# gerbenvoshol/fqzcomp5

Hardware: AMD Instinct MI355X
Metric: input MB/s encode+decode, 100MB blocks, -3 and -5; bit-exact vs CPU (higher is better)
Workload: dtype u8

## Files before the change

fqzcomp5_amd/csrc/block.cpp:

```cpp
#include <atomic>
#include <cstdio>
#include <algorithm>
#include <cstdlib>
#include <cstring>
#include <exception>
#include <functional>
#include <thread>
#include <deque>
#include <memory>
#include <vector>

#include "../../include/fqz5_block.h"
#include "rans_codec.hpp"
#include "fqz_codec.hpp"
#include "seq_codec.hpp"
#include "seq_cm.h"
#include "lzp_codec.hpp"
#include "names.hpp"
#include "host_dec.hpp"
#include "rans_format.hpp"

namespace fqz5 {

GpuCtx &gpu();
// ... 1033 lines not shown
                DecompressReq r;
                r.h_in = hs;
                r.d_in = secs[i].in + 9;
                r.in_size = clen;
                r.out_cap = rsz;
                r.d_out = g.arena.alloc_n<uint8_t>(size_t(rsz) + 1);
                LzpDecReq z;
                z.d_in = r.d_out;
                z.d_out = secs[i].out;
                z.cap = ulen;
                lzp_rans.push_back(reqs.size());
                reqs.push_back(r);
                who.push_back(-1);
                lzd.push_back(z);
                who_lzp.push_back(i);
                continue;
            }
            if (h[0] != 0) continue;
            DecompressReq r;
            r.h_in = h + 9;
            r.d_in = secs[i].in + 9;
            r.in_size = clen;
            r.out_cap = ulen;
            r.d_out = secs[i].out;
            reqs.push_back(r);
            who.push_back(i);
        }
        const double t1 = now_ms();
        const int hmode = host_decode_mode();
        std::vector<int> fqz_kind(fqz.size(), host::CK_FQZ), fqz_src(fqz.size(), -1);
        for (size_t k = 0; k < fqz.size(); k++) {
            const FqzDecReq &f = fqz[k];
            uint32_t tl = 0;
            const int vk = varint_get(f.h_in, f.h_in + f.in_size, &tl);
            if (vk > 0 && size_t(vk) + 1 < f.in_size && (f.h_in[vk + 1] & 8u) && f.d_seq) {
                fqz_kind[k] = host::CK_FQZ_SEQ;
                for (size_t m = 0; m < seqd.size(); m++)
                    if (seqd[m].d_out == f.d_seq) fqz_src[k] = int(m);
            }
        }
        std::vector<uint64_t> chain_n;
        std::vector<int> chain_kind;
        for (const SeqDecReq &q : seqd) { chain_n.push_back(q.n); chain_kind.push_back(host::CK_SEQ); }
        for (size_t k = 0; k < fqz.size(); k++) { chain_n.push_back(fqz[k].out_cap); chain_kind.push_back(fqz_kind[k]); }
        const std::vector<char> on = host::place(hmode, chain_n, chain_kind, 0);
        std::vector<char> seq_on_host(on.begin(), on.begin() + seqd.size()),
                          fqz_on_host(on.begin() + seqd.size(), on.end());
        for (size_t k = 0; k < fqz.size(); k++)
            if (fqz_src[k] >= 0 && seq_on_host[size_t(fqz_src[k])]) fqz_on_host[k] = 1;
        g_chains_host += uint64_t(std::count(seq_on_host.begin(), seq_on_host.end(), 1) +
                                  std::count(fqz_on_host.begin(), fqz_on_host.end(), 1));
        g_chains_gpu += uint64_t(std::count(seq_on_host.begin(), seq_on_host.end(), 0) +
                                 std::count(fqz_on_host.begin(), fqz_on_host.end(), 0));
        struct HostChain { uint8_t *buf = nullptr; size_t cap = 0, n = 0; int sec = -1; bool ok = false; };
        std::vector<HostChain> hc;
        std::vector<size_t> hc_idx;
        std::vector<int> hc_kind;
        for (size_t k = 0; k < seqd.size(); k++) {
            if (!seq_on_host[k]) continue;
            HostChain c;
            c.cap = c.n = seqd[k].n;
            c.buf = g.staging.alloc(c.cap + 1);
            c.sec = who_seq[k];
            hc.push_back(c);
            hc_idx.push_back(k);
            hc_kind.push_back(host::CK_SEQ);
        }
        for (size_t k = 0; k < fqz.size(); k++) {
            if (!fqz_on_host[k]) continue;
            HostChain c;
            c.cap = fqz[k].out_cap;
            c.buf = g.staging.alloc(c.cap + 1);
            c.sec = who_fqz[k];
            hc.push_back(c);
            hc_idx.push_back(k);
            hc_kind.push_back(fqz_kind[k]);
        }
        auto timed = [](int kind, bool gpu, uint64_t n, const std::function<bool()> &fn) {
            const double a = now_ns();
            const bool ok = fn();
            if (ok) host::measured(kind, gpu, n, now_ns() - a);
            return ok;
        };
        host::Jobs hjobs;
        std::vector<size_t> early_h;
        for (size_t j = 0; j < hc.size(); j++)
            if (hc_kind[j] != host::CK_FQZ_SEQ) early_h.push_back(j);
        hjobs.start(early_h.size(), [&](size_t t) {
            const size_t j = early_h[t];
            HostChain &c = hc[j];
            if (hc_kind[j] == host::CK_SEQ) {
                const SeqDecReq &q = seqd[hc_idx[j]];
                c.ok = timed(host::CK_SEQ, false, q.n, [&] {
                    return host::seq_decode(seq_h[hc_idx[j]], q.in_size, q.lens, q.nrec, q.both, q.k,
                                            c.buf, q.n) == 0;
                });
            } else {
                const FqzDecReq &f = fqz[hc_idx[j]];
                c.ok = timed(host::CK_FQZ, false, c.cap, [&] {
                    return host::fqz_decode(f.h_in, f.in_size, c.buf, c.cap, &c.n, nullptr, 0, nullptr, 0) == 0;
                });
            }
        });
        double t_names_up = 0;
        GpuCtx *gn = nullptr;
        std::unique_ptr<HedgeShare> nshare;
        host::Task tn;
        if (!nd.empty()) {
            gn = &gpu_aux(AUX_NAMES);
            nshare = std::make_unique<HedgeShare>(size_t(g.cus));
            tn = on_ctx(*gn, "decode_sections", t0, [&] {
                names_decode_batch(*gn, nd, [&](size_t k) {
                    if (nd[k].ok && nd[k].u_len)
                        FQZ5_HIP(hipMemcpyAsync(secs[who_name[k]].out, nd[k].names,
                                                nd[k].u_len, hipMemcpyHostToDevice, gn->stream));
                });
                gn->sync();
                if (trace) t_names_up = now_ms();
            });
        }
        std::vector<FqzDecReq> fqz_early;
        std::vector<size_t> early_of;
        std::vector<char> is_early(fqz.size(), 0);
        uint64_t early_longest = 0;
        for (size_t k = 0; k < fqz.size(); k++) {
            if (fqz_on_host[k] || fqz_kind[k] == host::CK_FQZ_SEQ) continue;
            fqz_early.push_back(fqz[k]);
            early_of.push_back(k);
            is_early[k] = 1;
            early_longest = std::max<uint64_t>(early_longest, fqz[k].out_cap);
        }
        GpuCtx *gf = nullptr;
        host::Task tf;
        if (!fqz_early.empty()) {
            gf = &gpu_aux(AUX_FQZ);
            tf = on_ctx(*gf, "decode_sections", t0, [&] {
                timed(host::CK_FQZ, true, early_longest, [&] { fqz_decode_batch(*gf, fqz_early); return true; });
            });
        }
        std::vector<SeqDecReq> seq_gpu;
        std::vector<size_t> seq_gpu_of;
        uint64_t seq_longest = 0;
        for (size_t m = 0; m < seqd.size(); m++)
            if (!seq_on_host[m]) {
                seq_gpu.push_back(seqd[m]);
                seq_gpu_of.push_back(m);
                seq_longest = std::max<uint64_t>(seq_longest, seqd[m].n);
            }
        GpuCtx *gs = nullptr;
        host::Task ts;
        if (!seq_gpu.empty()) {
            gs = &gpu_aux(AUX_SEQ0);
            ts = on_ctx(*gs, "decode_sections", t0, [&] {
                timed(host::CK_SEQ, true, seq_longest, [&] { seq_decode_batch(*gs, seq_gpu); return true; });
            });
        }
        host::CoreBudget cores;
        cores.core_ns.assign(size_t(host::threads()) - std::min(size_t(host::threads()), hjobs.running()), 0.0);
        decompress_batch(g, reqs, &cores);
        const double t_rans = trace ? now_ms() : 0;
        if (trace)
            std::fprintf(stderr, "decode_sections: %zu bytes to host in %.1f ms, rANS %.1f ms\n", tot,
                         t1 - t0, now_ms() - t1);
        if (!lzd.empty()) {
            std::vector<LzpDecReq> run;
            std::vector<int> run_who;
            for (size_t k = 0; k < lzd.size(); k++) {
                const DecompressReq &r = reqs[lzp_rans[k]];
                if (!r.ok) continue;
                lzd[k].in_len = r.out_size;
                run.push_back(lzd[k]);
                run_who.push_back(who_lzp[k]);
            }
            lzp_decode_batch(g, run);
            for (size_t k = 0; k < run.size(); k++) {
                fqz5_section_result &R = res[run_who[k]];
                R.status = run[k].ok ? 0 : -1;
                R.usize = run[k].out_len;
            }
        }
        ts.join();
        for (size_t i = 0; i < seq_gpu.size(); i++) seqd[seq_gpu_of[i]] = seq_gpu[i];
        {
            std::vector<FqzDecReq> late;
            std::vector<size_t> late_of;
            uint64_t longest = 0;
            for (size_t k = 0; k < fqz.size(); k++)
                if (!is_early[k] && !fqz_on_host[k]) {
                    late.push_back(fqz[k]);
                    late_of.push_back(k);
                    longest = std::max<uint64_t>(longest, fqz[k].out_cap);
                }
            if (!late.empty()) {
                timed(host::CK_FQZ_SEQ, true, longest, [&] { fqz_decode_batch(g, late); return true; });
                for (size_t k = 0; k < late.size(); k++) fqz[late_of[k]] = late[k];
            }
        }
        tf.join();
        for (size_t k = 0; k < fqz_early.size(); k++) fqz[early_of[k]] = fqz_early[k];
        if (!hc.empty()) {
            hjobs.join();
            std::vector<std::vector<const uint8_t *>> recp(hc.size());
            for (size_t j = 0; j < hc.size(); j++) {
                if (hc_kind[j] != host::CK_FQZ_SEQ) continue;
                const FqzDecReq &f = fqz[hc_idx[j]];
                const uint8_t *bases = nullptr;
                bool host_src = false;
                for (size_t m = 0; m < hc.size(); m++)
                    if (hc_kind[m] == host::CK_SEQ && secs[hc[m].sec].out == f.d_seq) {
                        bases = hc[m].ok ? hc[m].buf : nullptr;
                        host_src = true;
                    }
                uint64_t nb = 0;
                for (int r = 0; r < f.nrec; r++) nb += f.lens[r];
                if (!bases) {
                    uint8_t *b = g.staging.alloc(nb + 1);
                    if (!host_src) g.download(b, f.d_seq, nb);
                    else std::memset(b, 0, nb + 1);
                    bases = b;
                }
                recp[j].resize(size_t(std::max(f.nrec, 1)));
                uint64_t o = 0;
                for (int r = 0; r < f.nrec; r++) {
                    recp[j][size_t(r)] = bases + o;
                    o += f.lens[r];
                }
            }
            g.sync();
            host::Jobs hb;
            std::vector<size_t> late;
            for (size_t j = 0; j < hc.size(); j++)
                if (hc_kind[j] == host::CK_FQZ_SEQ) late.push_back(j);
            hb.start(late.size(), [&](size_t t) {
                HostChain &c = hc[late[t]];
                const FqzDecReq &f = fqz[hc_idx[late[t]]];
                c.ok = timed(host::CK_FQZ_SEQ, false, c.cap, [&] {
                    return host::fqz_decode(f.h_in, f.in_size, c.buf, c.cap, &c.n, nullptr, 0,
                                            recp[late[t]].data(), f.nrec) == 0;
                });
            });
            hb.join();
            for (HostChain &c : hc) {
                fqz5_section_result &R = res[c.sec];
                R.status = c.ok ? 0 : -1;
                R.usize = uint32_t(c.n);
                if (c.ok && c.n)
                    FQZ5_HIP(hipMemcpyAsync(secs[c.sec].out, c.buf, c.n, hipMemcpyHostToDevice, g.stream));
            }
        }
        const double t_hc = trace ? now_ms() : 0;
        tn.join();
        nshare.reset();
        const double t_nj = trace ? now_ms() : 0;
        for (size_t k = 0; k < nd.size(); k++) {
            fqz5_section_result &R = res[who_name[k]];
            if (!nd[k].ok) continue;
            R.status = 0;
            R.usize = nd[k].u_len;
        }
        for (size_t k = 0; k < reqs.size(); k++) {
            if (who[k] < 0) continue;
            fqz5_section_result &R = res[who[k]];
            R.status = reqs[k].ok ? 0 : -1;
            R.usize = reqs[k].out_size;
        }
        for (size_t k = 0; k < seqd.size(); k++) {
            if (seq_on_host[k]) continue;
            fqz5_section_result &R = res[who_seq[k]];
            R.status = seqd[k].ok ? 0 : -1;
            R.usize = seqd[k].n;
        }
        for (size_t k = 0; k < fqz.size(); k++) {
            if (fqz_on_host[k]) continue;
            fqz5_section_result &R = res[who_fqz[k]];
            R.status = fqz[k].ok ? 0 : -1;
            R.usize = uint32_t(fqz[k].out_size);
        }
        g.reset();
        if (gn) gn->reset();
        if (gf) gf->reset();
        if (gs) gs->reset();
        if (trace) {
            std::fprintf(stderr, "decode_sections: from its start: rANS done %.1f, host chains joined "
                         "%.1f, names uploaded %.1f, names joined %.1f, reset %.1f ms\n", t_rans - t0,
                         t_hc - t0, t_names_up ? t_names_up - t0 : -1.0, t_nj - t0, now_ms() - t0);
        }
        return 0;
    } catch (const std::exception &e) {
        fqz5_set_error(e.what());
        try { gpu().reset(); } catch (...) {}
        try { gpu_aux_reset_all(); } catch (...) {}
        return -1;
    }
}

}
```

fqzcomp5_amd/csrc/host_sched.cpp:

```cpp
#include <sched.h>
#include <algorithm>
#include <cstdlib>

#include "../../include/fqz5_mi355x.h"
#include "host_sched.hpp"

namespace fqz5 {
namespace host {

namespace {
constexpr double HOST_RANS_O0_NS = 1.0, HOST_RANS_O1_NS = 1.4;
constexpr double HOST_RANS_ENC_O0_NS = 0.65, HOST_RANS_ENC_O1_NS = 0.85;
std::atomic<double> g_ns[CK_N][2] = {{{30.0}, {330.0}}, {{16.0}, {180.0}}, {{24.0}, {400.0}},
                                     {{HOST_RANS_O0_NS}, {13.6}}, {{HOST_RANS_O1_NS}, {18.4}},
                                     {{HOST_RANS_ENC_O0_NS}, {4.6}}, {{HOST_RANS_ENC_O1_NS}, {4.6}}};
}

double chain_ns(int kind, bool gpu) { return g_ns[kind][gpu ? 1 : 0].load(std::memory_order_relaxed); }

void chain_measured(int kind, bool gpu, double ns) {
    if (!(ns > 0.0) || kind < 0 || kind >= CK_N) return;
    std::atomic<double> &a = g_ns[kind][gpu ? 1 : 0];
    double cur = a.load(std::memory_order_relaxed);
    while (!a.compare_exchange_weak(cur, 0.5 * cur + 0.5 * ns, std::memory_order_relaxed)) {}
// ... 38 lines not shown
}

std::vector<char> place(int mode, const std::vector<uint64_t> &n, const std::vector<int> &kind,
                        uint64_t min_n, const std::vector<double> *core_ns, std::vector<double> *committed) {
    std::vector<char> on(n.size(), 0);
    if (mode == 0 || (core_ns && core_ns->empty())) return on;
    if (mode != 2) {
        for (size_t i = 0; i < on.size(); i++) on[i] = mode == 1 || i % 2 == 0;
        return on;
    }
    std::vector<size_t> at;
    std::vector<uint64_t> ln;
    std::vector<int> lk;
    for (size_t i = 0; i < n.size(); i++)
        if (n[i] >= min_n) { at.push_back(i); ln.push_back(n[i]); lk.push_back(kind[i]); }
    const std::vector<char> p = plan(ln, lk, core_ns ? int(core_ns->size()) : threads(), core_ns, committed);
    for (size_t k = 0; k < at.size(); k++) on[at[k]] = p[k];
    return on;
}

int cores_of_rank() {
    int n = 0;
    cpu_set_t set;
    CPU_ZERO(&set);
    if (sched_getaffinity(0, sizeof set, &set) == 0) n = CPU_COUNT(&set);
    if (n <= 0) n = int(std::max(1u, std::thread::hardware_concurrency()));
    if (const char *e = std::getenv("LOCAL_WORLD_SIZE")) {
        const int w = std::atoi(e);
        if (w > 1) n /= w;
    }
    if (const char *e = std::getenv("OMP_NUM_THREADS")) {
        const int o = std::atoi(e);
        if (o > 0) n = std::min(n, o);
    }
    return std::max(1, n);
}

int threads() {
    static const int n = [] {
        if (const char *e = std::getenv("FQZ5_HOST_THREADS")) return std::max(1, std::atoi(e));
        return std::min(16, cores_of_rank());
    }();
    return n;
}

bool step_trace() {
    static const bool on = std::getenv("FQZ5_STEP_TRACE") != nullptr;
    return on;
}

void Jobs::start(size_t n, std::function<void(size_t)> fn, size_t max_threads, size_t grain, size_t callers) {
    fn_ = std::move(fn);
    n_ = n;
    grain_ = std::max<size_t>(grain, 1);
    next_ = 0;
    size_t t = std::min((n + grain_ - 1) / grain_, size_t(threads()));
    if (max_threads) t = std::min(t, max_threads);
    for (size_t k = callers; k < t; k++) th_.emplace_back([this] { work(); });
}

void Jobs::work() noexcept {
    for (size_t i; (i = next_.fetch_add(grain_)) < n_;) {
        try {
            for (size_t k = i; k < std::min(n_, i + grain_); k++) fn_(k);
        } catch (...) {
            std::lock_guard<std::mutex> lk(mu_);
            if (!err_) err_ = std::current_exception();
        }
    }
}

void Jobs::join() {
    for (auto &t : th_) t.join();
    th_.clear();
    std::exception_ptr e;
    std::swap(e, err_);
    if (e) std::rethrow_exception(e);
}

Jobs::~Jobs() {
    for (auto &t : th_) t.join();
}

void parallel_for(size_t n, const std::function<void(size_t)> &fn, size_t grain, size_t serial_below) {
    if (n < serial_below || threads() == 1) {
        for (size_t i = 0; i < n; i++) fn(i);
        return;
    }
    Jobs j;
    j.start(n, fn, 0, grain, 1);
    j.work();
    j.join();
}

}
}

extern "C" void fqz5_host_plan(const uint64_t *n, const int *kind, int count, int threads,
                               const double *core_ns, char *on_host) {
    using namespace fqz5;
    const std::vector<uint64_t> nv(n, n + count);
    const std::vector<int> kv(kind, kind + count);
    std::vector<double> cores;
    if (core_ns) cores.assign(core_ns, core_ns + threads);
    const std::vector<char> on = host::plan(nv, kv, threads, core_ns ? &cores : nullptr);
    std::copy(on.begin(), on.end(), on_host);
}
```

fqzcomp5_amd/csrc/host_sched.hpp:

```cpp
#pragma once
#include <time.h>
#include <atomic>
#include <chrono>
#include <cstddef>
#include <cstdint>
#include <exception>
#include <functional>
#include <memory>
#include <mutex>
#include <thread>
#include <utility>
#include <vector>

namespace fqz5 {
namespace host {

int threads();
int cores_of_rank();

enum ChainKind { CK_SEQ = 0, CK_FQZ = 1, CK_FQZ_SEQ = 2, CK_RANS_O0 = 3, CK_RANS_O1 = 4,
                 CK_RANS_ENC_O0 = 5, CK_RANS_ENC_O1 = 6, CK_N };
double chain_ns(int kind, bool gpu);
void chain_measured(int kind, bool gpu, double ns_per_symbol);
std::vector<char> plan(const std::vector<uint64_t> &n, const std::vector<int> &kind, int threads,
                       const std::vector<double> *core_ns = nullptr,
                       std::vector<double> *committed = nullptr);

constexpr uint64_t CHAIN_MIN = 1u << 20;
void measured(int kind, bool gpu, uint64_t n, double ns);

std::vector<char> place(int mode, const std::vector<uint64_t> &n, const std::vector<int> &kind,
                        uint64_t min_n, const std::vector<double> *core_ns = nullptr,
                        std::vector<double> *committed = nullptr);

struct CoreBudget {
    std::vector<double> core_ns;
};

class Jobs {
  public:
    void start(size_t n, std::function<void(size_t)> fn, size_t max_threads = 0, size_t grain = 1,
               size_t callers = 0);
    void work() noexcept;
    void join();
    size_t running() const { return th_.size(); }
    ~Jobs();

  private:
    std::function<void(size_t)> fn_;
    size_t n_ = 0, grain_ = 1;
    std::atomic<size_t> next_{0};
    std::mutex mu_;
    std::exception_ptr err_;
    std::vector<std::thread> th_;
};

class Task {
  public:
    Task() = default;
    explicit Task(std::function<void()> fn) {
        if (!fn) return;
        err_ = std::make_unique<std::exception_ptr>();
        th_ = std::thread([fn = std::move(fn), e = err_.get()] {
            try {
                fn();
            } catch (...) {
                *e = std::current_exception();
            }
        });
    }
    Task(Task &&) = default;
    Task &operator=(Task &&o) {
        wait();
        err_ = std::move(o.err_);
        th_ = std::move(o.th_);
        return *this;
    }
    bool running() const { return th_.joinable(); }
    void join() {
        wait();
        if (err_ && *err_) std::rethrow_exception(std::exchange(*err_, nullptr));
    }
    ~Task() { wait(); }

  private:
    void wait() { if (th_.joinable()) th_.join(); }
    std::unique_ptr<std::exception_ptr> err_;
    std::thread th_;
};

void parallel_for(size_t n, const std::function<void(size_t)> &fn, size_t grain, size_t serial_below);

bool step_trace();
inline double now_ns() {
    return std::chrono::duration<double, std::nano>(
               std::chrono::steady_clock::now().time_since_epoch()).count();
}
inline double now_ms() { return now_ns() * 1e-6; }
inline double thread_cpu_ns() {
    timespec t;
    if (clock_gettime(CLOCK_THREAD_CPUTIME_ID, &t)) return 0;
    return double(t.tv_sec) * 1e9 + double(t.tv_nsec);
}

}
}
```

fqzcomp5_amd/csrc/names.cpp:

```cpp
#include <algorithm>
#include <condition_variable>
#include <cstdio>
#include <cstdlib>
#include <cstring>
#include <exception>
#include <mutex>
#include <thread>

#include "host_lzp.hpp"
#include "names.hpp"
#include "rans_format.hpp"

namespace fqz5 {

namespace {
void put32(uint8_t *p, uint32_t v) { std::memcpy(p, &v, 4); }
uint32_t get32(const uint8_t *p) { uint32_t v; std::memcpy(&v, p, 4); return v; }

void on_threads(size_t n, const std::function<void(size_t)> &fn) { host::parallel_for(n, fn, 1, 2); }
using host::now_ms;
using host::step_trace;
}

void name_prepare(const uint8_t *h, uint32_t name_len, int strat, int level, NameEnc &E,
                  bool pipelined) {
    name_split(h, name_len, strat, level, E);
    name_tokenise(E, pipelined, nullptr);
}

void name_tokenise(NameEnc &E, bool pipelined, const T3Found *found) {
    if (E.strat == 0) return;
    E.tok_ok = tok3_tokenise(E.ids.data(), int(E.ids.size()), E.level, 0, E.tok, pipelined, found);
}

void name_split(const uint8_t *h, uint32_t name_len, int strat, int level, NameEnc &E) {
    E = NameEnc();
    E.strat = strat;
    E.level = level;
    E.name_len = name_len;
    if (strat == 0) return;
    if (strat == 1) {
        E.ids.assign(h, h + name_len);
        return;
    }
    E.ids.resize(name_len + 1);
    E.comments.resize(name_len + 1);
    char *cp1 = E.ids.data(), *cp2 = E.comments.data();
    const char *nb = reinterpret_cast<const char *>(h);
    uint32_t i = 0;
    while (i < name_len) {
        uint32_t j, w1end = 0, w2start = 0, w2end = 0;
        int f = 0;
        for (j = i; j < name_len; j++) {
            if (nb[j] == '\0') {
                w2end = j;
                break;
            }
            if (!w2start && (nb[j] == ' ' || nb[j] == '\t')) {
                w1end = j;
                w2start = j + 1;
                f |= 4;
            }
        }
        if (!w1end) w1end = j;
        if (!w2end) w2end = j;
        if (w2start) f |= nb[w2start - 1] == ' ' ? 0 : 8;
        if (w1end > 1 && nb[w1end - 2] == '/') {
            if (nb[w1end - 1] == '1') f |= 1, w1end -= 2;
            else if (nb[w1end - 1] == '2') f |= 3, w1end -= 2;
        }
        E.flag.push_back(uint8_t(f));
        std::memcpy(cp1, nb + i, w1end - i);
        cp1[w1end - i] = 0;
        cp1 += w1end - i + 1;
        if (w2start) {
            std::memcpy(cp2, nb + w2start, w2end - w2start);
            cp2[w2end - w2start] = 0;
            cp2 += w2end - w2start + 1;
        }
        i = j + 1;
    }
    E.ids.resize(size_t(cp1 - E.ids.data()));
    E.comments.resize(size_t(cp2 - E.comments.data()));
}
// ... 376 lines not shown
    D.flags.assign(u_lenf, 0);
    while (cp < cp_end) {
        while (cp1 < cp1_end && cp < cp_end && *cp1) *cp++ = *cp1++;
        cp1++;
        int flag = 0;
        if (cpf < cpf_end) flag = *cpf++;
        if ((flag & 1) && cp + 1 < cp_end) {
            *cp++ = '/';
            *cp++ = (flag & 2) ? '2' : '1';
        }
        if ((flag & 4) && cp < cp_end) *cp++ = (flag & 8) ? '\t' : ' ';
        if (cp2) {
            while (cp2 < cp2_end && cp < cp_end && *cp2) *cp++ = *cp2++;
            cp2++;
        }
        if (rec < int(u_lenf)) D.flags[size_t(rec)] = (flag & 3) == 3 ? 128u : 0u;
        rec++;
        if (cp == last_cp) break;
        if (cp < cp_end) *cp++ = 0;
        else return;
        last_cp = cp;
    }
    D.nrec = rec;
    if (cp < D.names + D.u_len) std::memset(cp, 0, size_t(D.names + D.u_len - cp));
    D.ok = true;
}

void name_dec_finish(GpuCtx &g, NameDec &D, const std::vector<DecompressReq> &reqs,
                     const std::vector<LzpDecReq> &lz) {
    name_dec_fetch(g, D, reqs, lz);
    name_dec_rebuild(D);
}

namespace {
void names_decode_batch_gpu(GpuCtx &g, std::vector<NameDec> &jobs,
                            const std::function<void(size_t)> &block_done) {
    const double t0 = step_trace() ? now_ms() : 0;
    std::vector<DecompressReq> reqs;
    std::vector<char> good(jobs.size());
    for (size_t k = 0; k < jobs.size(); k++) {
        good[k] = name_dec_parse(jobs[k]);
        if (good[k]) name_dec_add_requests(g, jobs[k], reqs);
    }
    if (!reqs.empty()) decompress_batch(g, reqs);
    std::vector<LzpDecReq> lz;
    for (size_t k = 0; k < jobs.size(); k++)
        if (good[k]) name_dec_add_lzp(g, jobs[k], reqs, lz);
    if (!lz.empty()) lzp_decode_batch(g, lz);
    const double t1 = step_trace() ? now_ms() : 0;
    for (size_t k = 0; k < jobs.size(); k++)
        if (good[k]) name_dec_fetch(g, jobs[k], reqs, lz);
        else jobs[k].fetched = false;
    const double t2 = step_trace() ? now_ms() : 0;
    on_threads(jobs.size(), [&](size_t k) { name_dec_rebuild(jobs[k]); });
    if (step_trace())
        std::fprintf(stderr, "names decode: %zu sections, %zu rANS streams + lzp %.1f ms, "
                     "fetch %.1f ms, rebuild %.1f ms\n", jobs.size(), reqs.size(), t1 - t0,
                     t2 - t1, now_ms() - t2);
    if (block_done)
        for (size_t k = 0; k < jobs.size(); k++) block_done(k);
}
}

void names_decode_batch(GpuCtx &g, std::vector<NameDec> &jobs,
                        const std::function<void(size_t)> &block_done) {
    if (host_decode_mode() == 0) {
        names_decode_batch_gpu(g, jobs, block_done);
        return;
    }
    const double t0 = now_ms();
    std::vector<DecompressReq> reqs;
    std::vector<char> good(jobs.size());
    for (size_t k = 0; k < jobs.size(); k++) {
        good[k] = name_dec_parse(jobs[k]);
        if (good[k]) name_dec_add_requests(g, jobs[k], reqs);
    }
    if (!reqs.empty()) decompress_batch(g, reqs);
    const double t1 = now_ms();
    struct Events {
        std::vector<hipEvent_t> ev;
        ~Events() { for (hipEvent_t e : ev) if (e) (void)hipEventDestroy(e); }
    } evs;
    evs.ev.assign(jobs.size(), nullptr);
    std::mutex mu;
    std::condition_variable cv;
    std::vector<size_t> finished;
    std::exception_ptr err;
    std::vector<double> t_fetch(jobs.size(), 0), t_done(jobs.size(), 0);
    for (size_t k = 0; k < jobs.size(); k++) {
        jobs[k].fetched = false;
        if (!good[k]) continue;
        name_dec_fetch_start(g, jobs[k], reqs);
        FQZ5_HIP(hipEventCreateWithFlags(&evs.ev[k], hipEventDisableTiming));
        FQZ5_HIP(hipEventRecord(evs.ev[k], g.stream));
    }
    host::Jobs tasks;
    tasks.start(jobs.size(), [&](size_t k) {
        NameDec &D = jobs[k];
        try {
            if (D.fetched) {
                FQZ5_HIP(hipEventSynchronize(evs.ev[k]));
                t_fetch[k] = now_ms();
                name_dec_rebuild(D);
            }
        } catch (...) {
            D.ok = false;
            std::lock_guard<std::mutex> lk(mu);
            if (!err) err = std::current_exception();
        }
        t_done[k] = now_ms();
        std::lock_guard<std::mutex> lk(mu);
        finished.push_back(k);
        cv.notify_one();
    });
    for (size_t seen = 0; seen < jobs.size();) {
        std::vector<size_t> now;
        {
            std::unique_lock<std::mutex> lk(mu);
            cv.wait(lk, [&] { return !finished.empty(); });
            now.swap(finished);
        }
        seen += now.size();
        if (block_done)
            for (size_t k : now) block_done(k);
    }
    tasks.join();
    if (err) std::rethrow_exception(err);
    if (step_trace()) {
        double f0 = 0, f1 = 0, d0 = 0, d1 = 0, ul = 0, rb = 0;
        uint64_t lz_c = 0, lz_i = 0, lz_o = 0;
        for (size_t k = 0; k < jobs.size(); k++) {
            if (t_fetch[k]) {
                f0 = f0 ? std::min(f0, t_fetch[k]) : t_fetch[k];
                f1 = std::max(f1, t_fetch[k]);
            }
            d0 = d0 ? std::min(d0, t_done[k]) : t_done[k];
            d1 = std::max(d1, t_done[k]);
            ul = std::max(ul, jobs[k].ms_unlzp);
            rb = std::max(rb, jobs[k].ms_rebuild);
            if (jobs[k].ok && jobs[k].lz_in) {
                lz_c += jobs[k].strat == 0 ? jobs[k].c_len : jobs[k].clen2;
                lz_i += jobs[k].lz_in_len;
                lz_o += jobs[k].strat == 0 ? jobs[k].u_len : jobs[k].out2_len;
            }
        }
        std::fprintf(stderr, "names decode: %zu sections, %zu rANS streams %.1f ms; from the call's "
                     "start: blocks fetched %.1f .. %.1f ms, complete %.1f .. %.1f ms (a host task "
                     "per block: the longest unlzp %.1f ms, the longest rebuild %.1f ms; lzp streams "
                     "%llu B coded, %llu B after rANS, %llu B expanded)\n",
                     jobs.size(), reqs.size(), t1 - t0, f0 ? f0 - t0 : 0.0, f1 ? f1 - t0 : 0.0,
                     d0 ? d0 - t0 : 0.0, d1 ? d1 - t0 : 0.0, ul, rb,
                     (unsigned long long)lz_c, (unsigned long long)lz_i, (unsigned long long)lz_o);
    }
}

}
```

fqzcomp5_amd/csrc/rans_decompress.cpp:

```cpp
#include <atomic>
#include <cstdio>
#include <cstdlib>
#include <algorithm>
#include <climits>
#include <cstring>

#include "host_rans.hpp"
#include "kernels.h"
#include "rans_codec.hpp"
#include "rans_format.hpp"

namespace fqz5 {

namespace {

struct DJ {
    const uint8_t *h = nullptr;
    const uint8_t *d = nullptr;
    uint32_t len = 0;
    uint32_t n = 0;
    bool o1 = false;
    int nx = 4;
    uint8_t *d_out = nullptr;
    int bits = 12;
// ... 229 lines not shown
    return on;
}

static bool o1reg_decoder() {
    static const bool on = [] {
        const char *e = std::getenv("FQZ5_O1REG");
        return e && e[0] == '1';
    }();
    return on;
}
static bool o1_keys(const DJ &j, DecJob &d) {
    const uint32_t rows = uint32_t(j.alpha.size()), M = 1u << j.bits;
    if (j.bits > 12 || rows > (j.bits == 12 ? 8u : 16u)) return false;
    const uint32_t rowsh = j.bits == 12 ? 29u : 28u;
    uint32_t nk = 0;
    for (uint32_t r = 0; r < rows; r++) {
        const uint32_t *F = &j.F[size_t(r) * 256];
        uint32_t x = 0;
        for (uint32_t s = 0; s < 256; s++) {
            if (!F[s]) continue;
            const auto it = std::lower_bound(j.alpha.begin(), j.alpha.end(), uint8_t(s));
            if (it == j.alpha.end() || *it != s || nk >= DEC_O1KEY_MAX || F[s] > M) return false;
            const uint32_t sym = uint32_t(it - j.alpha.begin());
            d.okey[nk++] = r << rowsh | x << 16 | (0xffffu - ((F[s] - 1) << 4 | sym));
            x += F[s];
        }
        if (x != M) return false;
    }
    if (!nk) return false;
    const uint32_t nk16 = (nk + 15) & ~15u;
    for (uint32_t k = nk; k < nk16; k++) d.okey[k] = d.okey[0];
    d.okeys = nk16;
    d.rowsh = rowsh;
    return true;
}

using host::now_ms;
using host::now_ns;
using host::step_trace;

std::atomic<uint64_t> g_rans_host{0}, g_rans_gpu{0};
std::atomic<uint64_t> g_dec_variant[DV_COUNT], g_dec_variant_hedged[DV_COUNT];

inline int chain_kind(const DJ &j) { return j.o1 ? host::CK_RANS_O1 : host::CK_RANS_O0; }

void Decompressor::run_djs(const std::vector<int> &ids, bool may_host) {
    for (int id : ids) {
        DJ &j = djs_[id];
        if (!j.ok || !j.n) continue;
        if (j.len < j.tab_len + 4u * j.nx) { j.ok = false; continue; }
        const uint8_t *s = j.h + j.tab_len;
        for (int z = 0; z < j.nx && j.ok; z++, s += 4) {
            const uint32_t x = s[0] | uint32_t(s[1]) << 8 | uint32_t(s[2]) << 16 | uint32_t(s[3]) << 24;
            if (x < (1u << 15)) j.ok = false;
        }
    }
    struct HostChain { int id; uint8_t *buf; bool ok; double ns; };
    std::vector<HostChain> hc;
    std::vector<char> on_host(djs_.size(), 0);
    size_t host_threads = 0;
    const int hmode = may_host ? host_decode_mode() : 0;
    if (hmode) {
        std::vector<int> el;
        for (int id : ids) {
            const DJ &j = djs_[id];
            if (!j.ok || !j.n || j.nx != 4 || j.len < j.tab_len + 16u) continue;
            el.push_back(id);
        }
        host_threads = cores_ ? cores_->core_ns.size() : size_t(host::threads());
        std::vector<uint64_t> n;
        std::vector<int> kind;
        for (int id : el) { n.push_back(djs_[id].n); kind.push_back(chain_kind(djs_[id])); }
        const std::vector<char> on = host::place(hmode, n, kind, host::CHAIN_MIN,
                                                 cores_ ? &cores_->core_ns : nullptr);
        for (size_t k = 0; k < el.size(); k++) on_host[el[k]] = on[k];
        for (int id : el)
            if (on_host[id]) hc.push_back({id, g_.staging.alloc(size_t(djs_[id].n) + 1), false, 0.0});
        auto cost = [&](const HostChain &c) {
            return double(djs_[c.id].n) * host::chain_ns(chain_kind(djs_[c.id]), false);
        };
        std::stable_sort(hc.begin(), hc.end(),
                         [&](const HostChain &a, const HostChain &b) { return cost(a) > cost(b); });
    }
    host::Jobs hjobs;
    hjobs.start(hc.size(), [&](size_t k) {
        HostChain &c = hc[k];
        const DJ &j = djs_[c.id];
        const double a = now_ns();
        const uint8_t *in = j.h + j.tab_len;
        const size_t in_len = j.len - j.tab_len;
        if (j.o1) {
            const uint32_t rows = uint32_t(j.alpha.size());
            c.ok = host::rans_dec_o1(j.F.data(), j.alpha.data(), rows, j.bits,
                                     dec_table_mode(true, rows, j.bits) == DEC_TAB_SPLIT, in, in_len,
                                     c.buf, j.n);
        } else {
            c.ok = host::rans_dec_o0(j.F.data(), j.bits, in, in_len, c.buf, j.n);
        }
        c.ns = now_ns() - a;
    }, host_threads);
    auto finish_host = [&] {
        if (hc.empty()) return;
        const double t0 = now_ms();
        hjobs.join();
        host_join_ms_ += now_ms() - t0;
        host_chains_ += hc.size();
        for (HostChain &c : hc) {
            DJ &j = djs_[c.id];
            host_longest_ms_ = std::max(host_longest_ms_, c.ns * 1e-6);
            if (!c.ok) { starved(j); continue; }
            host::measured(chain_kind(j), false, j.n, c.ns);
            FQZ5_HIP(hipMemcpyAsync(j.d_out, c.buf, j.n, hipMemcpyHostToDevice, g_.stream));
        }
    };
    g_rans_host += hc.size();

    std::vector<uint32_t> tabs;
    std::vector<uint8_t> alphas;
    struct Off { size_t tab, alpha; };
    std::vector<Off> offs;
    std::vector<int> used;
    for (int id : ids) {
        DJ &j = djs_[id];
        if (!j.ok || !j.n || on_host[id]) continue;
        const size_t rows = j.o1 ? j.alpha.size() : 1;
        const uint32_t mode = dec_table_mode(j.o1, uint32_t(rows), j.bits);
        Off o{tabs.size(), alphas.size()};
        tabs.resize(tabs.size() + dec_tab_words(mode, uint32_t(rows), j.bits), 0);
        if (j.o1) alphas.insert(alphas.end(), j.alpha.begin(), j.alpha.end());
        offs.push_back(o);
        used.push_back(id);
    }
    host_parallel(used.size(), [&](size_t k) {
        DJ &j = djs_[used[k]];
        const uint32_t M = 1u << j.bits;
        const size_t rows = j.o1 ? j.alpha.size() : 1;
        const uint32_t mode = dec_table_mode(j.o1, uint32_t(rows), j.bits);
        uint32_t *t = &tabs[offs[k].tab];
        uint8_t *tsym = reinterpret_cast<uint8_t *>(t);
        uint32_t *tfb = t + rows * M / 4;
        const uint32_t rpl = dec_rp_log(uint32_t(rows));
        for (size_t r = 0; r < rows; r++) {
            const uint32_t *F = &j.F[r * 256];
            uint32_t x = 0;
            for (int s = 0; s < 256; s++) {
                if (!F[s]) continue;
                uint32_t sym = s;
                if (j.o1) {
                    auto it = std::lower_bound(j.alpha.begin(), j.alpha.end(), uint8_t(s));
                    if (it == j.alpha.end() || *it != s) { j.ok = false; break; }
                    sym = uint32_t(it - j.alpha.begin());
                }
                if (mode == DEC_TAB_SPLIT) tfb[(r << rpl) + sym] = ((F[s] - 1) << 16) | x;
                for (uint32_t y = 0; y < F[s] && x + y < M; y++) {
                    if (mode == DEC_TAB_SPLIT)
                        tsym[r * M + x + y] = uint8_t(sym);
                    else
                        t[r * M + x + y] = ((F[s] - 1) << (j.bits + 8)) | (y << 8) | sym;
                }
                x += F[s];
            }
        }
    });
    if (used.empty()) {
        finish_host();
        return;
    }
    const uint32_t *d_tabs = g_.upload(tabs);
    const uint8_t *d_alpha = alphas.empty() ? nullptr : g_.upload(alphas);
    int32_t *d_status = g_.arena.alloc_n<int32_t>(used.size());
    g_.memset0(d_status, used.size() * 4);
    std::vector<DecJob> djs;
    uint32_t lds = 0;
    std::vector<size_t> ord;
    for (size_t k = 0; k < used.size(); k++) {
        DJ &j = djs_[used[k]];
        if (j.len < j.tab_len + 4u * j.nx) { j.ok = false; continue; }
        ord.push_back(k);
    }
    std::stable_sort(ord.begin(), ord.end(), [&](size_t a, size_t b) {
        return djs_[used[a]].n / djs_[used[a]].nx > djs_[used[b]].n / djs_[used[b]].nx;
    });
    double bytes = 0;
    for (size_t k : ord) {
        DJ &j = djs_[used[k]];
        const uint32_t rows = j.o1 ? uint32_t(j.alpha.size()) : 1u;
        const uint32_t mode = dec_table_mode(j.o1, rows, j.bits);
        djs.push_back(DecJob{j.d + j.tab_len, d_tabs + offs[k].tab,
                             j.o1 ? d_alpha + offs[k].alpha : nullptr, j.d_out, d_status + k,
                             j.len - j.tab_len, j.n, j.nx, j.bits, rows, mode, nullptr, 0, {}});
        if (!j.o1 && j.nx == 4 && reg_decoder()) {
            DecJob &d = djs.back();
            uint32_t k2 = 0, x = 0;
            for (int s = 0; s < 256 && k2 <= DEC_REG_MAX; s++) {
                if (!j.F[s]) continue;
                if (k2 < DEC_REG_MAX) d.reg[k2] = x | (j.F[s] << 16);
                k2++;
                x += j.F[s];
            }
            if (k2 >= 1 && k2 <= DEC_REG_MAX && x == (1u << j.bits)) d.nreg = k2;
        }
        if (j.o1 && j.nx == 4 && o1reg_decoder() && o1_keys(j, djs.back()))
            lds = std::max(lds, DEC_O1REG_LDS_BYTES);
        bytes += double(j.n) + (j.len - j.tab_len);
        lds = std::max(lds, dec_lds_bytes(rows, j.bits, int(mode)));
    }
    EventPair ev((g_.prof.on || prof_on()) && !ord.empty(), g_.stream);
    static const double tabw = [] {
        const char *e = std::getenv("FQZ5_HEDGE_TABW");
        return e ? std::atof(e) : 1.0;
    }();
    std::vector<double> steps;
    for (const DecJob &d : djs)
        steps.push_back(double(d.n / uint32_t(d.nx)) * (d.nreg ? 1.0 : tabw));
    HedgeShare share(size_t(g_.cus));
    const std::vector<int> cp = hedge_plan(steps, share.cus);
    for (size_t k = 0; k < djs.size(); k++) {
        const int v = dec_variant(djs[k]);
        g_dec_variant[v].fetch_add(1, std::memory_order_relaxed);
        if (cp[k] > 1) g_dec_variant_hedged[v].fetch_add(1, std::memory_order_relaxed);
    }
    if (std::any_of(cp.begin(), cp.end(), [](int c) { return c > 1; })) {
        const size_t nj = djs.size();
        uint32_t *d_done = g_.arena.alloc_n<uint32_t>(nj);
        g_.memset0(d_done, nj * 4);
        for (size_t k = 0; k < nj; k++) djs[k].done = d_done + k;
        const std::vector<int> pos = xcd_grouping() ? xcd_layout(cp, share.cus)
                                                    : std::vector<int>();
        if (!pos.empty()) {
            std::vector<DecJob> laid(pos.size());
            for (size_t i = 0; i < pos.size(); i++) {
                if (pos[i] >= 0) laid[i] = djs[size_t(pos[i])];
                else { laid[i] = djs[0]; laid[i].nx = 0; }
            }
            djs.swap(laid);
        } else {
            for (size_t k = 0; k < nj; k++)
                for (int c = 1; c < cp[k]; c++) djs.push_back(djs[k]);
        }
    }
    lds = g_.chain_lds(lds, djs.size());
    g_rans_gpu += ord.size();
    const double launch_t0 = now_ns();
    if (!djs.empty()) FQZ5_HIP(launch_dec(g_.upload(djs), int(djs.size()), lds, g_.stream));
    ev.stop(g_.stream);
    std::vector<int32_t> st(used.size());
    g_.download(st.data(), d_status, st.size());
    g_.sync();
    if (!ord.empty()) {
        const DJ &lj = djs_[used[ord[0]]];
        if (lj.nx == 4) host::measured(chain_kind(lj), true, lj.n, now_ns() - launch_t0);
    }
    finish_host();
    if (ev.on) {
        const double ms = ev.ms();
        g_.prof.dec_ms += ms;
        g_.prof.dec_launches += 1;
        g_.prof.dec_bytes += bytes;
        if (prof_on()) prof_add(PK_RANS_DEC, ms, bytes);
    }
    for (size_t k = 0; k < used.size(); k++)
        if (st[k]) starved(djs_[used[k]]);
}

void Decompressor::starved(DJ &j) {
    std::vector<uint8_t> buf(size_t(j.n) + 1);
    j.ok = host::rans_dec_ref(j.h, j.len, buf.data(), j.n, j.o1, j.nx);
    if (!j.ok) return;
    FQZ5_HIP(hipMemcpyAsync(j.d_out, buf.data(), j.n, hipMemcpyHostToDevice, g_.stream));
    g_.sync();
}

void Decompressor::run(std::vector<DecompressReq> &reqs) {
    const double t0 = step_trace() ? now_ms() : 0;
    std::vector<int> roots;
    for (auto &r : reqs) {
        r.ok = false;
        r.out_size = 0;
        roots.push_back(parse(r.h_in, r.d_in, r.in_size, r.d_out, r.out_cap, 0));
    }
    const double t1 = step_trace() ? now_ms() : 0;
    std::vector<int> hdr;
    for (size_t i = 0; i < djs_.size(); i++)
        if (djs_[i].hdr_dj >= 0) hdr.push_back(djs_[i].hdr_dj);
    if (!hdr.empty()) {
        run_djs(hdr, false);
        for (size_t i = 0; i < djs_.size(); i++) {
            DJ &j = djs_[i];
            if (j.hdr_dj < 0) continue;
            DJ &hj = djs_[j.hdr_dj];
            if (!hj.ok) { j.ok = false; continue; }
            j.hdr.resize(hj.n);
            g_.download(j.hdr.data(), hj.d_out, hj.n);
        }
        g_.sync();
        for (size_t i = 0; i < djs_.size(); i++) {
            DJ &j = djs_[i];
            if (j.hdr_dj < 0 || !j.ok) continue;
            j.ok = parse_o1_table(j, j.hdr.data(), j.hdr.data() + j.hdr.size());
        }
    }
    std::vector<int> rest;
    std::vector<char> is_hdr(djs_.size(), 0);
    for (int h : hdr) is_hdr[h] = 1;
    for (size_t i = 0; i < djs_.size(); i++)
        if (!is_hdr[i]) rest.push_back(int(i));
    const double t2 = step_trace() ? now_ms() : 0;
    run_djs(rest, true);
    const double t3 = step_trace() ? now_ms() : 0;

    std::vector<CopyItem> cps;
    for (auto &N : nodes_) {
        if (N.stripe || !N.ok) continue;
        if (N.dj_main >= 0 && !djs_[N.dj_main].ok) N.ok = false;
        if (N.dj_meta >= 0 && !djs_[N.dj_meta].ok) N.ok = false;
        if (N.d_cat)
            for (uint32_t o = 0; o < N.ent_n; o += 65536)
                cps.push_back({N.d_cat + o, N.d_ent + o, std::min<uint32_t>(65536, N.ent_n - o), 0});
    }
    if (!cps.empty()) FQZ5_HIP(launch_copy(g_.upload(cps), int(cps.size()), g_.stream));

    std::vector<int> rl;
    std::vector<const uint8_t *> probes;
    for (size_t i = 0; i < nodes_.size(); i++) {
        Node &N = nodes_[i];
        if (!N.stripe && N.ok && N.rle) {
            if (!N.meta_len || N.osz == UINT32_MAX) { N.ok = false; continue; }
            rl.push_back(int(i));
        }
    }
    if (!rl.empty()) {
        std::vector<std::vector<uint8_t>> mh(rl.size());
        for (size_t k = 0; k < rl.size(); k++) {
            Node &N = nodes_[rl[k]];
            uint32_t m = std::min<uint32_t>(N.meta_len, 257);
            mh[k].resize(m);
// ... 194 lines not shown
```

Baseline: 4373.

## Upload host-decoded chains as each finishes on a second stream

Adds a JobsAsDone helper that hands out host job indices as they complete. Decode paths in block.cpp and rans_decompress use it to issue each host-to-device copy on a forked second stream the moment its chain finishes, instead of after all host jobs join. In rans decompress, host work completion is now polled while the GPU kernel runs, so host uploads overlap the GPU decode. The GPU timing sample is taken when the stream query first reports done. It adds mutex/condvar traffic and stream fork/join overhead, and failed chains are deferred to the end.

```diff
diff --git a/fqzcomp5_amd/csrc/block.cpp b/fqzcomp5_amd/csrc/block.cpp
--- a/fqzcomp5_amd/csrc/block.cpp
+++ b/fqzcomp5_amd/csrc/block.cpp
@@ -1139,7 +1139,7 @@
             if (ok) host::measured(kind, gpu, n, now_ns() - a);
             return ok;
         };
-        host::Jobs hjobs;
+        host::JobsAsDone hjobs;
         std::vector<size_t> early_h;
         for (size_t j = 0; j < hc.size(); j++)
             if (hc_kind[j] != host::CK_FQZ_SEQ) early_h.push_back(j);
@@ -1256,6 +1256,16 @@
         tf.join();
         for (size_t k = 0; k < fqz_early.size(); k++) fqz[early_of[k]] = fqz_early[k];
         if (!hc.empty()) {
+            g.fork();
+            auto chain_done = [&](size_t j) {
+                const HostChain &c = hc[j];
+                fqz5_section_result &R = res[c.sec];
+                R.status = c.ok ? 0 : -1;
+                R.usize = uint32_t(c.n);
+                if (c.ok && c.n)
+                    FQZ5_HIP(hipMemcpyAsync(secs[c.sec].out, c.buf, c.n, hipMemcpyHostToDevice, g.stream2));
+            };
+            hjobs.each_done([&](size_t t) { chain_done(early_h[t]); });
             hjobs.join();
             std::vector<std::vector<const uint8_t *>> recp(hc.size());
             for (size_t j = 0; j < hc.size(); j++) {
@@ -1284,10 +1294,10 @@
                 }
             }
             g.sync();
-            host::Jobs hb;
             std::vector<size_t> late;
             for (size_t j = 0; j < hc.size(); j++)
                 if (hc_kind[j] == host::CK_FQZ_SEQ) late.push_back(j);
+            host::JobsAsDone hb;
             hb.start(late.size(), [&](size_t t) {
                 HostChain &c = hc[late[t]];
                 const FqzDecReq &f = fqz[hc_idx[late[t]]];
@@ -1296,14 +1306,9 @@
                                             recp[late[t]].data(), f.nrec) == 0;
                 });
             });
+            hb.each_done([&](size_t t) { chain_done(late[t]); });
             hb.join();
-            for (HostChain &c : hc) {
-                fqz5_section_result &R = res[c.sec];
-                R.status = c.ok ? 0 : -1;
-                R.usize = uint32_t(c.n);
-                if (c.ok && c.n)
-                    FQZ5_HIP(hipMemcpyAsync(secs[c.sec].out, c.buf, c.n, hipMemcpyHostToDevice, g.stream));
-            }
+            g.join();
         }
         const double t_hc = trace ? now_ms() : 0;
         tn.join();
diff --git a/fqzcomp5_amd/csrc/host_sched.cpp b/fqzcomp5_amd/csrc/host_sched.cpp
--- a/fqzcomp5_amd/csrc/host_sched.cpp
+++ b/fqzcomp5_amd/csrc/host_sched.cpp
@@ -144,6 +144,44 @@
     for (auto &t : th_) t.join();
 }
 
+void JobsAsDone::start(size_t n, std::function<void(size_t)> fn, size_t max_threads) {
+    n_ = n;
+    taken_ = 0;
+    ended_.clear();
+    jobs_.start(n, [this, fn = std::move(fn)](size_t i) {
+        struct Ended {
+            JobsAsDone &s;
+            size_t i;
+            ~Ended() {
+                std::lock_guard<std::mutex> lk(s.mu_);
+                s.ended_.push_back(i);
+                s.cv_.notify_one();
+            }
+        } ended{*this, i};
+        fn(i);
+    }, max_threads);
+}
+
+void JobsAsDone::each_done(const std::function<void(size_t)> &done, const std::function<bool()> &idle) {
+    bool watch = bool(idle);
+    while (taken_ < n_) {
+        std::vector<size_t> now;
+        {
+            std::unique_lock<std::mutex> lk(mu_);
+            const auto some = [&] { return !ended_.empty(); };
+            while (watch && !cv_.wait_for(lk, std::chrono::microseconds(IDLE_US), some)) {
+                lk.unlock();
+                watch = idle();
+                lk.lock();
+            }
+            cv_.wait(lk, some);
+            now.swap(ended_);
+        }
+        taken_ += now.size();
+        for (size_t k : now) done(k);
+    }
+}
+
 void parallel_for(size_t n, const std::function<void(size_t)> &fn, size_t grain, size_t serial_below) {
     if (n < serial_below || threads() == 1) {
         for (size_t i = 0; i < n; i++) fn(i);
diff --git a/fqzcomp5_amd/csrc/host_sched.hpp b/fqzcomp5_amd/csrc/host_sched.hpp
--- a/fqzcomp5_amd/csrc/host_sched.hpp
+++ b/fqzcomp5_amd/csrc/host_sched.hpp
@@ -2,6 +2,7 @@
 #include <time.h>
 #include <atomic>
 #include <chrono>
+#include <condition_variable>
 #include <cstddef>
 #include <cstdint>
 #include <exception>
@@ -55,6 +56,23 @@
     std::vector<std::thread> th_;
 };
 
+class JobsAsDone {
+  public:
+    static constexpr int IDLE_US = 200;
+    void start(size_t n, std::function<void(size_t)> fn, size_t max_threads = 0);
+    void each_done(const std::function<void(size_t)> &done,
+                   const std::function<bool()> &idle = nullptr);
+    void join() { jobs_.join(); }
+    size_t running() const { return jobs_.running(); }
+
+  private:
+    std::mutex mu_;
+    std::condition_variable cv_;
+    std::vector<size_t> ended_;
+    size_t n_ = 0, taken_ = 0;
+    Jobs jobs_;
+};
+
 class Task {
   public:
     Task() = default;
diff --git a/fqzcomp5_amd/csrc/names.cpp b/fqzcomp5_amd/csrc/names.cpp
--- a/fqzcomp5_amd/csrc/names.cpp
+++ b/fqzcomp5_amd/csrc/names.cpp
@@ -1,5 +1,4 @@
 #include <algorithm>
-#include <condition_variable>
 #include <cstdio>
 #include <cstdlib>
 #include <cstring>
@@ -542,10 +541,6 @@
         ~Events() { for (hipEvent_t e : ev) if (e) (void)hipEventDestroy(e); }
     } evs;
     evs.ev.assign(jobs.size(), nullptr);
-    std::mutex mu;
-    std::condition_variable cv;
-    std::vector<size_t> finished;
-    std::exception_ptr err;
     std::vector<double> t_fetch(jobs.size(), 0), t_done(jobs.size(), 0);
     for (size_t k = 0; k < jobs.size(); k++) {
         jobs[k].fetched = false;
@@ -554,7 +549,7 @@
         FQZ5_HIP(hipEventCreateWithFlags(&evs.ev[k], hipEventDisableTiming));
         FQZ5_HIP(hipEventRecord(evs.ev[k], g.stream));
     }
-    host::Jobs tasks;
+    host::JobsAsDone tasks;
     tasks.start(jobs.size(), [&](size_t k) {
         NameDec &D = jobs[k];
         try {
@@ -565,27 +560,13 @@
             }
         } catch (...) {
             D.ok = false;
-            std::lock_guard<std::mutex> lk(mu);
-            if (!err) err = std::current_exception();
+            t_done[k] = now_ms();
+            throw;
         }
         t_done[k] = now_ms();
-        std::lock_guard<std::mutex> lk(mu);
-        finished.push_back(k);
-        cv.notify_one();
     });
-    for (size_t seen = 0; seen < jobs.size();) {
-        std::vector<size_t> now;
-        {
-            std::unique_lock<std::mutex> lk(mu);
-            cv.wait(lk, [&] { return !finished.empty(); });
-            now.swap(finished);
-        }
-        seen += now.size();
-        if (block_done)
-            for (size_t k : now) block_done(k);
-    }
+    tasks.each_done([&](size_t k) { if (block_done) block_done(k); });
     tasks.join();
-    if (err) std::rethrow_exception(err);
     if (step_trace()) {
         double f0 = 0, f1 = 0, d0 = 0, d1 = 0, ul = 0, rb = 0;
         uint64_t lz_c = 0, lz_i = 0, lz_o = 0;
diff --git a/fqzcomp5_amd/csrc/rans_decompress.cpp b/fqzcomp5_amd/csrc/rans_decompress.cpp
--- a/fqzcomp5_amd/csrc/rans_decompress.cpp
+++ b/fqzcomp5_amd/csrc/rans_decompress.cpp
@@ -335,7 +335,8 @@
         std::stable_sort(hc.begin(), hc.end(),
                          [&](const HostChain &a, const HostChain &b) { return cost(a) > cost(b); });
     }
-    host::Jobs hjobs;
+    if (!hc.empty()) g_.fork();
+    host::JobsAsDone hjobs;
     hjobs.start(hc.size(), [&](size_t k) {
         HostChain &c = hc[k];
         const DJ &j = djs_[c.id];
@@ -352,19 +353,23 @@
         }
         c.ns = now_ns() - a;
     }, host_threads);
-    auto finish_host = [&] {
+    auto finish_host = [&](const std::function<bool()> &gpu_busy) {
         if (hc.empty()) return;
         const double t0 = now_ms();
+        std::vector<size_t> failed;
+        hjobs.each_done([&](size_t k) {
+            HostChain &c = hc[k];
+            DJ &j = djs_[c.id];
+            host_longest_ms_ = std::max(host_longest_ms_, c.ns * 1e-6);
+            if (!c.ok) { failed.push_back(k); return; }
+            host::measured(chain_kind(j), false, j.n, c.ns);
+            FQZ5_HIP(hipMemcpyAsync(j.d_out, c.buf, j.n, hipMemcpyHostToDevice, g_.stream2));
+        }, gpu_busy);
         hjobs.join();
         host_join_ms_ += now_ms() - t0;
         host_chains_ += hc.size();
-        for (HostChain &c : hc) {
-            DJ &j = djs_[c.id];
-            host_longest_ms_ = std::max(host_longest_ms_, c.ns * 1e-6);
-            if (!c.ok) { starved(j); continue; }
-            host::measured(chain_kind(j), false, j.n, c.ns);
-            FQZ5_HIP(hipMemcpyAsync(j.d_out, c.buf, j.n, hipMemcpyHostToDevice, g_.stream));
-        }
+        g_.join();
+        for (size_t k : failed) starved(djs_[hc[k].id]);
     };
     g_rans_host += hc.size();
 
@@ -416,7 +421,7 @@
         }
     });
     if (used.empty()) {
-        finish_host();
+        finish_host(nullptr);
         return;
     }
     const uint32_t *d_tabs = g_.upload(tabs);
@@ -499,12 +504,18 @@
     ev.stop(g_.stream);
     std::vector<int32_t> st(used.size());
     g_.download(st.data(), d_status, st.size());
+    double launch_t1 = 0;
+    finish_host([&] {
+        if (hipStreamQuery(g_.stream) == hipErrorNotReady) return true;
+        launch_t1 = now_ns();
+        return false;
+    });
     g_.sync();
+    if (!launch_t1) launch_t1 = now_ns();
     if (!ord.empty()) {
         const DJ &lj = djs_[used[ord[0]]];
-        if (lj.nx == 4) host::measured(chain_kind(lj), true, lj.n, now_ns() - launch_t0);
-    }
-    finish_host();
+        if (lj.nx == 4) host::measured(chain_kind(lj), true, lj.n, launch_t1 - launch_t0);
+    }
     if (ev.on) {
         const double ms = ev.ms();
         g_.prof.dec_ms += ms;
```

New measurement: 4123. -5.7%, worse.
